# csiro-crop-informatics/biokanga

Measured on AMD Instinct MI355X. Metric: aligned reads/s (SAM-identical) on 100 bp SE vs GRCh38, 1->8 MI355X, higher is better.
Workload: dtype u8

## Files before the change

### biokanga_amd/csrc/bk_ctx_int.h

```cpp
#pragma once
#include <atomic>
#include <thread>
#include <hip/hip_runtime.h>

#include <cstdio>
#include <cstring>
#include <functional>
#include <string>
#include <utility>
#include <vector>

#include "bk_device.h"
#include "bk_devbuf.h"
#include "bk_stage.h"

#define HIP_TRY(expr)                                                                              \
    do {                                                                                           \
        hipError_t e__ = (expr);                                                                   \
        if (e__ != hipSuccess) {                                                                   \
            fprintf(stderr, "biokanga_amd: %s failed: %s (%s:%d)\n", #expr, hipGetErrorString(e__), __FILE__, __LINE__); \
            return e__ == hipErrorOutOfMemory ? BK_ERR_MEM : BK_ERR_INTERNAL;                      \
        }                                                                                          \
    } while (0)
#define BK_TRY(expr) do { const int rc__ = (expr); if (rc__) return rc__; } while (0)
// ... 150 lines not shown
    bk_timing timing{};
    std::vector<hipEvent_t> ev_pool;
    std::vector<uint64_t> loci_offs;
    std::vector<bk_loci> loci;
    std::vector<bk_loci_trims> loci_trims;
    std::vector<bk_seg2> seg2;
};


namespace bk {
struct DevReads {
    const uint8_t *bases = nullptr;
    const uint64_t *offs = nullptr;
    const uint32_t *lens = nullptr;
    const uint32_t *words = nullptr;
    const bk_nbase *exc = nullptr;
    uint64_t n_exc = 0;
};
int engine_align_device(bk_ctx *c, const DevReads &in, uint32_t nreads, bk_hit *d_out, hipStream_t s, uint32_t maxlen_known = 0, uint32_t minlen_known = 0);
void release_swin(bk_ctx *c);
void drop_swin(bk_ctx *c);
int engine_pair_device(bk_ctx *c, const DevReads &in, uint32_t n_pairs, bk_hit *d_hits, uint32_t maxlen, const bk_pe_params *pe, hipStream_t s,
                       bk_seg2 *seg2_host = nullptr, bk_seg2 *seg2_dev = nullptr);
int engine_prepare_packed(bk_ctx *c, const uint16_t *d_lens16, uint32_t nreads, uint64_t n_words, const bk_nbase *d_exc, uint64_t n_exc,
                          uint32_t *d_lens32, uint64_t *d_offs, uint32_t *maxlen, uint32_t *minlen, hipStream_t s);
}

namespace bk {
hipError_t dev_zero_now(void *p, size_t bytes);
int upload_host(void *d_dst, const void *h_src, size_t bytes, int device);
int upload_file(void *d_dst, int fd, uint64_t file_ofs, size_t bytes, int device);
bool host_is_pinned(const void *p);

std::vector<uint32_t> seq_len_by_id(const bk_ctx *c);
void gather_split(uint64_t total_bytes, uint32_t n, const std::function<void(uint32_t, uint32_t)> &part);
template <class SpanOf> inline void gather_reads(uint8_t *dst, const uint64_t *dst_ofs, const uint8_t *src, uint64_t total_bytes, uint32_t n, SpanOf span_of)
{
    gather_split(total_bytes, n, [&](uint32_t lo, uint32_t hi) {
        for (uint32_t t = lo; t < hi; t++) {
            if (dst_ofs[t] == ~0ULL) continue;
            const std::pair<uint64_t, uint32_t> sp = span_of(t);
            memcpy(dst + dst_ofs[t], src + sp.first, sp.second);
        }
    });
}
}
```

### biokanga_amd/csrc/bk_engine.cpp

```cpp
#include "bk_engine_int.h"
#include "bk_iv_slot.h"
#include "bk_wave_form.h"

namespace bk {
int size_heavy_scratch(bk_ctx *c)
{
    int slides = std::max(1, (c->cfg.slides_per100 * c->max_read_len + 99) / 100);
    uint64_t worst = c->cfg.max_iter ? (uint64_t)slides * (uint64_t)c->cfg.max_iter : kNodeCap;
    if (worst > kNodeCap) worst = kNodeCap;
    uint32_t ts = 1024;
    while (ts < 2 * worst) ts <<= 1;
    uint32_t slots = 4096;
    while ((uint64_t)slots * ts * 8 > (16ULL << 30) && slots > 64) slots >>= 1;
    if (c->hs.htab && c->hs.tab_size == ts && c->hs.n_slots == slots) return BK_OK;
    BatchBufs &m = c->buf;
    m.htab.reset();
    m.slot_epoch.reset();
    c->hs = HeavyScratch{};
    HIP_TRY(m.htab.ensure((size_t)slots * ts));
    HIP_TRY(m.slot_epoch.ensure(slots));
    launch_fill_u64(m.htab.get(), (uint64_t)slots * ts, 0ULL, c->stream);
    HIP_TRY(hipGetLastError());
    HIP_TRY(hipMemsetAsync(m.slot_epoch.get(), 0, (size_t)slots * 4, c->stream));
    HIP_TRY(hipStreamSynchronize(c->stream));
// ... 668 lines not shown
        case Span::Prep: c->timing.ms_prep += m; c->timing.ms_other += m; break;
        case Span::Other: c->timing.ms_other += m; break;
        }
    }
    return BK_OK;
}


}

using namespace bk;

int bk::engine_align_device(bk_ctx *c, const DevReads &in, uint32_t nreads, bk_hit *d_out, hipStream_t s, uint32_t maxlen_known, uint32_t minlen_known)
{
    return align_device(c, in, nreads, d_out, s, maxlen_known, false, minlen_known);
}

namespace {
struct CastU64 {
    __host__ __device__ unsigned long long operator()(const uint32_t &v) const { return (unsigned long long)v; }
};
}

int bk::engine_prepare_packed(bk_ctx *c, const uint16_t *d_lens16, uint32_t nreads, uint64_t n_words, const bk_nbase *d_exc, uint64_t n_exc,
                              uint32_t *d_lens32, uint64_t *d_offs, uint32_t *maxlen, uint32_t *minlen, hipStream_t s)
{
    launch_widen_lens(d_lens16, nreads, d_lens32, (unsigned long long *)d_offs, s);
    HIP_TRY(hipGetLastError());
    size_t need = 0;
    HIP_TRY(bk::prim::exclusive_sum(nullptr, need, (unsigned long long *)d_offs, (unsigned long long *)d_offs, (size_t)nreads, s));
    if (need > c->buf.scan_tmp.cap()) {
        HIP_TRY(hipStreamSynchronize(s));
        HIP_TRY(c->buf.scan_tmp.ensure(need + 256));
    }
    size_t tb = c->buf.scan_tmp.cap();
    HIP_TRY(bk::prim::exclusive_sum(c->buf.scan_tmp.get(), tb, (unsigned long long *)d_offs, (unsigned long long *)d_offs, (size_t)nreads, s));
    HIP_TRY(hipMemsetAsync(c->fixed.ctr_aux.get(), 0, 32, s));
    launch_packed_extent(d_offs, d_lens32, nreads, c->fixed.ctr_aux.get(), s);
    launch_check_exc(d_exc, n_exc, d_lens32, nreads, reinterpret_cast<uint32_t *>(c->fixed.ctr_aux.get() + 2), s);
    launch_min_len(d_lens32, nreads, reinterpret_cast<uint32_t *>(c->fixed.ctr_aux.get() + 3), s);
    HIP_TRY(hipGetLastError());
    unsigned long long h[4] = {0, 0, 0, 0};
    HIP_TRY(hipMemcpyAsync(h, c->fixed.ctr_aux.get(), 32, hipMemcpyDeviceToHost, s));
    HIP_TRY(hipStreamSynchronize(s));
    if (h[0] != n_words || h[1] > (unsigned long long)kMaxReadLenAbs || (uint32_t)h[2] != 0) return BK_ERR_PARAMS;
    *maxlen = (uint32_t)h[1];
    *minlen = min_len_of((uint32_t)h[3]);
    return BK_OK;
}

int bk::engine_pair_device(bk_ctx *c, const DevReads &in, uint32_t n_pairs, bk_hit *d_hits, uint32_t maxlen, const bk_pe_params *pe, hipStream_t s,
                           bk_seg2 *seg2_host, bk_seg2 *seg2_dev)
{
    const uint32_t nreads = 2 * n_pairs;
    const uint32_t wpr = words_per_read(maxlen);
    const uint32_t ivc = c->cap_iv_cores ? c->cap_iv_cores : iv_cores_for(c, maxlen);
    BK_TRY(batch_scratch_or_release_swin(c, nreads, wpr, 0, ivc));
    const DevBatch b = make_batch(c, in, 0, nreads, wpr, c->cap_iv_cores, d_hits);
    if (c->params.min_chimeric_len > 0 && !seg2_host && !seg2_dev) return BK_ERR_PARAMS;
    bk_seg2 *d_seg2 = seg2_dev;
    if (!d_seg2 && seg2_host) {
        BK_TRY(ensure_seg2(c, nreads));
        d_seg2 = c->buf.seg2.get();
        HIP_TRY(hipMemcpyAsync(d_seg2, seg2_host, (size_t)nreads * sizeof(bk_seg2), hipMemcpyHostToDevice, s));
    }
    HIP_TRY(hipMemsetAsync(c->fixed.small.get(), 0, kSmallWords * 4, s));
    launch_pe(c->ix, c->cfg, b, pe->pe_mode, pe->pair_min_len, pe->pair_max_len, pe->pair_strand ? 1 : 0, d_hits, n_pairs,
              c->buf.heavy.get(), c->fixed.small.get() + kSmCount, c->h_small.get() + kSmCount, d_seg2, c->params.min_chimeric_len, maxlen > 512 ? 1 : 0, c->buf.chrom_accept.get(), c->n_chrom_accept, s);
    HIP_TRY(hipGetLastError());
    if (seg2_host && !seg2_dev) HIP_TRY(hipMemcpyAsync(seg2_host, d_seg2, (size_t)nreads * sizeof(bk_seg2), hipMemcpyDeviceToHost, s));
// ... 195 lines not shown
    for (unsigned t = 0; t < nt; t++) {
        for (const bk_nbase &e : found[t]) { if (total < exc_cap) exc[total] = e; total++; }
    }
    *n_exc = total;
    return total > exc_cap ? BK_ERR_MEM : BK_OK;
}

int bk_align_batch_packed(bk_ctx *c, const uint32_t *words, uint64_t n_words, const uint16_t *lens, uint32_t nreads, const bk_nbase *exc,
                          uint64_t n_exc, bk_hit *out)
{
    if (!c || (nreads && (!lens || !out)) || (n_words && !words) || (n_exc && !exc)) return BK_ERR_PARAMS;
    if (!nreads) return BK_OK;
    HIP_TRY(hipSetDevice(c->device));
    hipStream_t s = c->stream;
    static_assert(kPackedPadWords >= kNwLongest, "packed read words must be padded by the widest register-window family");
    BatchBufs &m = c->buf;
    HIP_TRY(m.in_words.ensure(n_words + kPackedPadWords));
    HIP_TRY(m.in_exc.ensure(n_exc));
    BK_TRY(ensure_in_reads(c, nreads, true));
    if (n_words) HIP_TRY(hipMemcpyAsync(m.in_words.get(), words, n_words * 4, hipMemcpyHostToDevice, s));
    HIP_TRY(hipMemcpyAsync(m.in_lens16.get(), lens, (size_t)nreads * 2, hipMemcpyHostToDevice, s));
    if (n_exc) HIP_TRY(hipMemcpyAsync(m.in_exc.get(), exc, n_exc * sizeof(bk_nbase), hipMemcpyHostToDevice, s));
    uint32_t maxlen = 0, minlen = 0;
    BK_TRY(engine_prepare_packed(c, m.in_lens16.get(), nreads, n_words, m.in_exc.get(), n_exc, m.in_lens.get(), m.in_offs.get(), &maxlen, &minlen, s));
    DevReads in;
    in.offs = m.in_offs.get(); in.lens = m.in_lens.get(); in.words = m.in_words.get(); in.exc = m.in_exc.get(); in.n_exc = n_exc;
    BK_TRY(align_device(c, in, nreads, m.in_out.get(), s));
    HIP_TRY(hipMemcpy(out, m.in_out.get(), (size_t)nreads * sizeof(bk_hit), hipMemcpyDeviceToHost));
    return BK_OK;
}

int bk_pair_batch(bk_ctx *c, const uint8_t *bases, const uint64_t *offs, const uint32_t *lens, uint32_t n_pairs, bk_hit *hits,
                  const bk_pe_params *pe)
{
    return bk_pair_batch_seg2(c, bases, offs, lens, n_pairs, hits, nullptr, pe);
}

int bk_pair_batch_seg2(bk_ctx *c, const uint8_t *bases, const uint64_t *offs, const uint32_t *lens, uint32_t n_pairs, bk_hit *hits,
                       bk_seg2 *seg2, const bk_pe_params *pe)
{
    if (!c || !pe || (n_pairs && (!bases || !offs || !lens || !hits))) return BK_ERR_PARAMS;
    if (c->params.min_chimeric_len > 0 && n_pairs && !seg2) return BK_ERR_PARAMS;
    if (pe->pe_mode < 1 || pe->pe_mode > 4 || pe->pair_min_len < 1 || pe->pair_max_len < pe->pair_min_len) return BK_ERR_PARAMS;
    if (!n_pairs) return BK_OK;
    if (n_pairs > 0x7fffffffu) return BK_ERR_PARAMS;
    HIP_TRY(hipSetDevice(c->device));
    const uint32_t nreads = 2 * n_pairs;
// ... 118 lines not shown
```

### biokanga_amd/csrc/bk_engine_int.h

```cpp
#pragma once
#include <hip/hip_runtime.h>
#include <fcntl.h>
#include <unistd.h>
#include "bk_prim.h"

#include <algorithm>
#include <cstdio>
#include <cstdlib>
#include <ctime>
#include <cstring>
#include <map>
#include <mutex>
#include <string>
#include <atomic>
#include <thread>
#include <type_traits>
#include <vector>

#include <dlfcn.h>
#include <rccl/rccl.h>

#include "bk_ctx_int.h"
#include "bk_phase_plan.h"
#include "bk_cpus.h"
#include "bk_wait.h"
#include "bk_env.h"
#include "sfx_file.h"


namespace bk {
void launch_pack_target(const uint8_t *seq, uint64_t n, uint64_t *tgt4, uint64_t nwords, hipStream_t s);
void launch_pack_target2(const uint64_t *tgt4, uint64_t nwords4, uint64_t *tgt2, unsigned int *nflag32, int flag_shift, hipStream_t s);
void launch_split_sa5(const uint8_t *sa5, uint64_t n, uint32_t *lo, uint8_t *hi, hipStream_t s);
void launch_build_ktab(const DevIndex &ix, void *tab, int k, bool tab64, hipStream_t s, uint64_t i0 = 0, uint64_t i1 = 0, unsigned long long *starts = nullptr, bool pairs = false);
void launch_fill_ktab2_y(void *tab2, const uint32_t *k2, uint64_t n_entries, hipStream_t s, const uint32_t *sa_elem = nullptr);
void launch_max_len(const uint32_t *lens, uint32_t n, uint32_t *out, hipStream_t s);
void launch_min_len(const uint32_t *lens, uint32_t n, uint32_t *out, hipStream_t s);
void launch_widen_lens(const uint16_t *lens16, uint32_t n, uint32_t *lens32, unsigned long long *nwords, hipStream_t s);
void launch_check_exc(const bk_nbase *exc, uint64_t n_exc, const uint32_t *lens, uint32_t n_reads, uint32_t *bad, hipStream_t s);
void launch_packed_extent(const uint64_t *offs, const uint32_t *lens, uint32_t n, unsigned long long *out, hipStream_t s);
void launch_snp_pileup(const DevIndex &ix, const uint8_t *bases, const uint64_t *offs, const uint32_t *id2idx, const bk_snp_aln *alns, uint64_t n_alns,
                       uint32_t *planes, hipStream_t s);
void launch_site_octamers(const DevIndex &ix, const bk_site_req *reqs, uint64_t n, int32_t rel_ofs, bk_site_res *out, hipStream_t s);
void launch_primer_correct(const DevIndex &ix, const bk_primer_req *reqs, uint64_t n, bk_primer_res *out, hipStream_t s);
void launch_snp_gather(const DevIndex &ix, const uint32_t *planes, uint64_t g0, uint32_t n, uint32_t *out, hipStream_t s);
void launch_snp_centroids(const DevIndex &ix, const uint32_t *planes, uint64_t g0, uint32_t chrom_len, uint32_t min_reads, uint32_t *hist, hipStream_t s);
void launch_snp_sites(const DevIndex &ix, const uint32_t *planes, uint64_t g0, uint32_t chrom_len, uint32_t min_reads, double min_prop,
                      bk_snp_site *sites, uint32_t cap, uint32_t *n_sites, unsigned long long *totals, hipStream_t s);
void launch_count_seqs(const bk_hit *out, uint32_t n, const uint32_t *id2idx, uint32_t n_ent, unsigned long long *counts, hipStream_t s);
void launch_fill_u64(unsigned long long *p, uint64_t n, unsigned long long v, hipStream_t s);
void launch_prep(const DevAlignCfg &cfg, const DevBatch &b, uint32_t *act, uint32_t *act_cnt, uint32_t *cmax, uint32_t *stage,
                 uint32_t *stripe_cnt, hipStream_t s, const PrepSearch0 *s0 = nullptr);
void launch_search(const DevIndex &ix, const DevAlignCfg &cfg, const DevBatch &b, const uint32_t *act, uint32_t n_act,
                   int phase, int cmax, int nstr, int lazy, hipStream_t s);
void launch_build_isa(const uint32_t *sa, uint64_t n, uint32_t *isa, hipStream_t s, uint64_t i0 = 0, uint64_t i1 = 0);
void launch_build_swin(const DevIndex &ix, void *swin, int words, hipStream_t s);
void launch_swin_breaks(const DevIndex &ix, const int *w, int n_levels, unsigned long long *const *brk, uint64_t a, uint64_t e, uint64_t n_words,
                        const unsigned long long *starts, hipStream_t s);
void launch_swin_cover(const unsigned long long *brk, uint64_t n, uint32_t max_run, uint32_t min_run, uint32_t *flags, uint64_t n_blocks, int first_level, hipStream_t s);
void launch_pack_ktab64(const uint64_t *tab, uint64_t n_entries, uint32_t *off, uint64_t *hi, uint32_t *overflow, hipStream_t s);
void launch_count_nonzero(const uint32_t *flags, uint64_t n, unsigned long long *count, hipStream_t s);
// ... 114 lines not shown
```

### biokanga_amd/csrc/bk_prep.hip

```cpp
#include "bk_dev_search_a.h"
#include "bk_plan_table.h"

namespace bk {


__global__ void __launch_bounds__(256) k_compact_lists(CompactJobs J)
{
    const int li = blockIdx.y;
    __shared__ uint32_t s_pre[kListStripes + 1];
    if (threadIdx.x < 64) {
        uint32_t run = 0;
        for (int s0 = 0; s0 < kListStripes; s0 += 64) {
            uint32_t v = J.set.cnt[(s0 + threadIdx.x) * 16 + li];
            for (int off = 1; off < 64; off <<= 1) { uint32_t u = __shfl_up(v, off); if ((int)threadIdx.x >= off) v += u; }
            s_pre[s0 + threadIdx.x + 1] = run + v;
            run += __shfl(v, 63);
        }
        if (threadIdx.x == 0) s_pre[0] = 0;
    }
    __syncthreads();
    const uint32_t tot = s_pre[kListStripes], old = *J.total[li];
    const uint32_t *__restrict__ stage = J.set.stage[li];
    uint32_t *__restrict__ dense = J.dense[li];
    for (uint32_t i = blockIdx.x * 256 + threadIdx.x; i < tot; i += gridDim.x * 256) {
// ... 146 lines not shown
            unsigned long long *p = reinterpret_cast<unsigned long long *>(b.rd4 + ((uint64_t)rr * 2 + st) * b.wpr + w);
            atomicAnd(p, ~m);
            atomicOr(p, code16 & m);
        }
    }
}

__global__ void __launch_bounds__(256) k_check_exc(const bk_nbase *__restrict__ exc, uint64_t n_exc, const uint32_t *__restrict__ lens, uint32_t n_reads,
                                                   uint32_t *__restrict__ bad)
{
    const uint64_t i = (uint64_t)blockIdx.x * blockDim.x + threadIdx.x;
    if (i >= n_exc) return;
    const bk_nbase e = exc[i];
    bool ok = e.read < n_reads && e.code >= 4 && e.code <= 7;
    if (ok) ok = (uint32_t)e.pos + e.run < lens[e.read];
    if (ok && i > 0) {
        const bk_nbase q = exc[i - 1];
        ok = q.read < e.read || (q.read == e.read && (uint32_t)q.pos + q.run < e.pos);
    }
    if (!ok) atomicAdd(bad, 1u);
}

__global__ void __launch_bounds__(256) k_widen_lens(const uint16_t *__restrict__ lens16, uint32_t n, uint32_t *__restrict__ lens32,
                                                    unsigned long long *__restrict__ nwords)
{
    const uint32_t i = blockIdx.x * blockDim.x + threadIdx.x;
    if (i >= n) return;
    const uint32_t l = lens16[i];
    lens32[i] = l;
    nwords[i] = (l + 15) >> 4;
}

__global__ void __launch_bounds__(256) k_packed_extent(const uint64_t *__restrict__ offs, const uint32_t *__restrict__ lens, uint32_t n,
                                                       unsigned long long *__restrict__ out)
{
    unsigned long long e = 0, l = 0;
    for (uint64_t i = (uint64_t)blockIdx.x * blockDim.x + threadIdx.x; i < n; i += (uint64_t)gridDim.x * blockDim.x) {
        const unsigned long long len = lens[i], end = offs[i] + ((len + 15) >> 4);
        e = end > e ? end : e;
        l = len > l ? len : l;
    }
    for (int off = 32; off > 0; off >>= 1) {
        const unsigned long long e2 = __shfl_down(e, off), l2 = __shfl_down(l, off);
        e = e2 > e ? e2 : e;
        l = l2 > l ? l2 : l;
    }
    if ((threadIdx.x & 63) == 0) {
        if (e) atomicMax(out + 0, e);
        if (l) atomicMax(out + 1, l);
    }
}

void launch_packed_extent(const uint64_t *offs, const uint32_t *lens, uint32_t n, unsigned long long *out, hipStream_t s)
{
    unsigned blocks = (n + 255) / 256;
    if (blocks > 2048) blocks = 2048;
    if (n) hipLaunchKernelGGL(k_packed_extent, dim3(blocks), dim3(256), 0, s, offs, lens, n, out);
}

void launch_widen_lens(const uint16_t *lens16, uint32_t n, uint32_t *lens32, unsigned long long *nwords, hipStream_t s)
{
    if (n) hipLaunchKernelGGL(k_widen_lens, dim3((n + 255) / 256), dim3(256), 0, s, lens16, n, lens32, nwords);
}

void launch_check_exc(const bk_nbase *exc, uint64_t n_exc, const uint32_t *lens, uint32_t n_reads, uint32_t *bad, hipStream_t s)
{
    if (n_exc) hipLaunchKernelGGL(k_check_exc, dim3((unsigned)((n_exc + 255) / 256)), dim3(256), 0, s, exc, n_exc, lens, n_reads, bad);
}

__global__ void __launch_bounds__(256) k_pack_reads(DevBatch b, const uint32_t *__restrict__ pairs, uint32_t n_pairs)
{
    const uint32_t wpr = b.wpr;
    const uint32_t per_read = 2 * wpr;
    const uint32_t rpb = 256 / per_read;
    const uint32_t lr = threadIdx.x / per_read;
    if (lr >= rpb) return;
    uint64_t r = (uint64_t)blockIdx.x * rpb + lr;
    if (pairs != nullptr) {
        if (r >= 2ULL * n_pairs) return;
        r = 2ULL * pairs[r >> 1] + (r & 1);
    }
    if (r >= b.n_reads) return;
    const uint32_t rem = threadIdx.x - lr * per_read;
    const uint32_t st = rem >= wpr ? 1 : 0, w = rem - st * wpr;
    int len = (int)b.lens[r];
// ... 505 lines not shown
```

### biokanga_amd/csrc/bk_stream.cpp

```cpp
#include <hip/hip_runtime.h>
#include "bk_prim.h"

#include <algorithm>
#include <cstdlib>
#include <condition_variable>
#include <deque>
#include <map>
#include <mutex>
#include <thread>

#include "bk_ctx_int.h"
#include "bk_wave_form.h"
#include "bk_wait.h"
#include "bk_env.h"

namespace {

struct CastU64 {
    __host__ __device__ unsigned long long operator()(const uint32_t &v) const { return (unsigned long long)v; }
};

__global__ void __launch_bounds__(256) k_extent(const uint64_t *__restrict__ offs, const uint32_t *__restrict__ lens, uint32_t n,
                                                unsigned long long nbases, unsigned long long *__restrict__ out)
{
// ... 25 lines not shown
    uint64_t ticket = 0;
    const uint8_t *bases = nullptr;
    uint64_t nbases = 0;
    const uint64_t *offs = nullptr;
    const uint32_t *lens = nullptr;
    const uint32_t *words = nullptr;
    uint64_t n_words = 0;
    const uint16_t *lens16 = nullptr;
    const bk_nbase *exc = nullptr;
    uint64_t n_exc = 0;
    uint32_t n = 0;
    bk_hit *out = nullptr;
    bool dev = false;
    const uint8_t *d_bases = nullptr;
    const uint64_t *d_offs = nullptr;
    const uint32_t *d_lens = nullptr;
    bk_hit *d_out = nullptr;
    hipEvent_t ev_in = nullptr;
    ~Job() { if (ev_in) (void)hipEventDestroy(ev_in); }
    int slot = 0;
    int rc = BK_OK;
    bool done = false;
    double t_submit = 0, t_done = 0;
    std::vector<uint64_t> loci_offs;
    std::vector<bk_loci> loci;
    std::vector<bk_loci_trims> loci_trims;
    std::vector<bk_seg2> seg2;
};

struct Slot {
    bk::DevBuf<uint8_t> d_bases;
    bk::DevBuf<uint16_t> d_lens16;
    bk::DevBuf<bk_nbase> d_exc;
    bk::DevBuf<uint64_t> d_offs;
    bk::DevBuf<uint32_t> d_lens;
    bk::DevBuf<bk_hit> d_out;
    hipEvent_t ev_up = nullptr, ev_al = nullptr;
};

using bk::now_s;

}

struct bk_stream {
    bk_ctx *ctx = nullptr;
    int depth = 0;
    uint32_t max_reads = 0;
    uint64_t max_bases = 0;
    uint64_t max_words = 0;
    std::vector<Slot> slots;
    hipStream_t s_up = nullptr, s_al = nullptr, s_dn = nullptr;
    bk::DevBuf<uint8_t> d_scan_tmp;
    size_t scan_tmp_bytes = 0;
    bk::DevBuf<unsigned long long> d_ext;
    bk::PinBuf<unsigned long long> h_ext;
    std::thread t_up, t_al, t_dn;
    hipEvent_t ev_w_al = nullptr, ev_w_dn = nullptr;
    std::mutex mu;
    std::condition_variable cv;
    std::deque<Job *> q_up, q_al, q_dn;
    std::map<uint64_t, Job *> jobs;
    uint64_t next_ticket = 1, n_done = 0;
    bool stop = false, list_modes = false, has_pe = false, span_open = false;
    bk_pe_params pe{};
    bk_stream_stats stats{};
    double t_first_submit = 0, t_last_done = 0;

    void fail(Job *j, int rc) { if (j->rc == BK_OK) j->rc = rc; }
    static int rc_of(hipError_t e) { return e == hipSuccess ? BK_OK : (e == hipErrorOutOfMemory ? BK_ERR_MEM : BK_ERR_INTERNAL); }

    Job *pop(std::deque<Job *> &q)
    {
        std::unique_lock<std::mutex> lk(mu);
        cv.wait(lk, [&] { return stop || !q.empty(); });
        if (q.empty()) return nullptr;
        Job *j = q.front();
        q.pop_front();
        return j;
    }
    void push(std::deque<Job *> &q, Job *j)
    {
        { std::lock_guard<std::mutex> lk(mu); q.push_back(j); }
        cv.notify_all();
    }

    void run_upload()
    {
        (void)hipSetDevice(ctx->device);
        while (Job *j = pop(q_up)) {
            Slot &sl = slots[j->slot];
            hipError_t e = hipSuccess;
            if (j->dev) { push(q_al, j); continue; }
            if (j->n && j->lens16) {
                const size_t wb = (size_t)j->n_words * 4;
                if (wb) {
                    if (bk::host_is_pinned(j->words)) e = hipMemcpyAsync(sl.d_bases.get(), j->words, wb, hipMemcpyHostToDevice, s_up);
                    else if (bk::upload_host(sl.d_bases.get(), j->words, wb, ctx->device) != BK_OK) e = hipErrorUnknown;
                }
                if (e == hipSuccess) e = hipMemcpyAsync(sl.d_lens16.get(), j->lens16, (size_t)j->n * 2, hipMemcpyHostToDevice, s_up);
                if (e == hipSuccess && j->n_exc > sl.d_exc.cap()) e = sl.d_exc.ensure(j->n_exc + j->n_exc / 4 + 1024);
                if (e == hipSuccess && j->n_exc) e = hipMemcpyAsync(sl.d_exc.get(), j->exc, (size_t)j->n_exc * sizeof(bk_nbase), hipMemcpyHostToDevice, s_up);
            } else if (j->n) {
                if (bk::host_is_pinned(j->bases)) e = hipMemcpyAsync(sl.d_bases.get(), j->bases, j->nbases, hipMemcpyHostToDevice, s_up);
                else if (bk::upload_host(sl.d_bases.get(), j->bases, j->nbases, ctx->device) != BK_OK) e = hipErrorUnknown;
                if (e == hipSuccess && j->offs) e = hipMemcpyAsync(sl.d_offs.get(), j->offs, (size_t)j->n * 8, hipMemcpyHostToDevice, s_up);
                if (e == hipSuccess) e = hipMemcpyAsync(sl.d_lens.get(), j->lens, (size_t)j->n * 4, hipMemcpyHostToDevice, s_up);
            }
            if (e == hipSuccess) e = hipEventRecord(sl.ev_up, s_up);
            if (e != hipSuccess) fail(j, rc_of(e));
            push(q_al, j);
        }
    }

    void run_align()
    {
        (void)hipSetDevice(ctx->device);
        const bool timing = bk::env::timing();
        double t_free = now_s();
        for (;;) {
            Job *j = pop(q_al);
            if (!j) break;
            const double t_got = now_s();
            double t_prep = t_got;
            Slot &sl = slots[j->slot];
            if (j->dev) {
                if (j->rc == BK_OK && j->n) {
                    hipError_t e = hipStreamWaitEvent(s_al, j->ev_in, 0);
                    bk::DevReads in;
                    in.bases = j->d_bases; in.offs = j->d_offs; in.lens = j->d_lens;
                    int rc = e == hipSuccess ? bk::engine_align_device(ctx, in, j->n, j->d_out, s_al, 0) : rc_of(e);
                    if (rc == BK_OK && has_pe) {
                        rc = bk::engine_pair_device(ctx, in, j->n / 2, j->d_out, (uint32_t)ctx->last_maxlen, &pe, s_al, ctx->seg2.empty() ? nullptr : ctx->seg2.data());
                    }
                    if (rc) fail(j, rc);
                    else if (list_modes) {
                        j->loci_offs.swap(ctx->loci_offs);
                        j->loci.swap(ctx->loci);
                        j->loci_trims.swap(ctx->loci_trims);
                        j->seg2.swap(ctx->seg2);
                    }
                }
                push(q_dn, j);
                t_free = now_s();
                continue;
            }
            if (j->rc == BK_OK && j->n && j->lens16) {
                hipError_t e = hipStreamWaitEvent(s_al, sl.ev_up, 0);
                uint32_t maxlen = 0, minlen = 0;
                int rc = e == hipSuccess ? bk::engine_prepare_packed(ctx, sl.d_lens16.get(), j->n, j->n_words, sl.d_exc.get(), j->n_exc, sl.d_lens.get(), sl.d_offs.get(), &maxlen, &minlen, s_al)
                                         : rc_of(e);
                t_prep = now_s();
                bk::DevReads in;
                in.offs = sl.d_offs.get(); in.lens = sl.d_lens.get(); in.words = reinterpret_cast<const uint32_t *>(sl.d_bases.get()); in.exc = sl.d_exc.get(); in.n_exc = j->n_exc;
                if (rc == BK_OK) rc = bk::engine_align_device(ctx, in, j->n, sl.d_out.get(), s_al, maxlen, minlen);
                if (rc == BK_OK && has_pe) rc = bk::engine_pair_device(ctx, in, j->n / 2, sl.d_out.get(), maxlen, &pe, s_al, ctx->seg2.empty() ? nullptr : ctx->seg2.data());
                if (rc) fail(j, rc);
                else if (list_modes) {
                    j->loci_offs.swap(ctx->loci_offs);
                    j->loci.swap(ctx->loci);
                    j->loci_trims.swap(ctx->loci_trims);
                    j->seg2.swap(ctx->seg2);
                }
                if (j->rc == BK_OK) {
                    e = hipEventRecord(sl.ev_al, s_al);
                    if (e != hipSuccess) fail(j, rc_of(e));
                }
            } else if (j->rc == BK_OK && j->n) {
                hipError_t e = hipStreamWaitEvent(s_al, sl.ev_up, 0);
                if (e == hipSuccess && !j->offs) {
                    size_t tb = scan_tmp_bytes;
                    rocprim::transform_iterator<const uint32_t *, CastU64, unsigned long long> in(sl.d_lens.get(), CastU64());
                    e = bk::prim::exclusive_sum(d_scan_tmp.get(), tb, in, (unsigned long long *)sl.d_offs.get(), (size_t)j->n, s_al);
                }
                if (e == hipSuccess) e = hipMemsetAsync(d_ext.get(), 0, 24, s_al);
                if (e == hipSuccess) {
                    unsigned blocks = (j->n + 255) / 256;
                    if (blocks > 2048) blocks = 2048;
                    hipLaunchKernelGGL(k_extent, dim3(blocks), dim3(256), 0, s_al, sl.d_offs.get(), sl.d_lens.get(), j->n, (unsigned long long)j->nbases, d_ext.get());
                    e = hipGetLastError();
                }
                if (e == hipSuccess) e = hipMemcpyAsync(h_ext.get(), d_ext.get(), 24, hipMemcpyDeviceToHost, s_al);
                if (e == hipSuccess) e = bk::wait_stream(s_al, ev_w_al);
                if (e != hipSuccess) fail(j, rc_of(e));
                else if (h_ext.get()[0] > j->nbases || h_ext.get()[1] > (unsigned long long)bk::kMaxReadLenAbs) fail(j, BK_ERR_PARAMS);
                const uint32_t maxlen = (uint32_t)h_ext.get()[1], minlen = bk::min_len_of((uint32_t)h_ext.get()[2]);
                if (j->rc == BK_OK) {
                    bk::DevReads in;
                    in.bases = sl.d_bases.get(); in.offs = sl.d_offs.get(); in.lens = sl.d_lens.get();
                    int rc = bk::engine_align_device(ctx, in, j->n, sl.d_out.get(), s_al, maxlen, minlen);
                    if (rc == BK_OK && has_pe) rc = bk::engine_pair_device(ctx, in, j->n / 2, sl.d_out.get(), maxlen, &pe, s_al, ctx->seg2.empty() ? nullptr : ctx->seg2.data());
                    if (rc) fail(j, rc);
                    else if (list_modes) {
                        j->loci_offs.swap(ctx->loci_offs);
                        j->loci.swap(ctx->loci);
                    j->loci_trims.swap(ctx->loci_trims);
                        j->seg2.swap(ctx->seg2);
                    }
                }
                if (j->rc == BK_OK) {
                    e = hipEventRecord(sl.ev_al, s_al);
                    if (e != hipSuccess) fail(j, rc_of(e));
                }
            }
            if (ctx->debug || timing)
                fprintf(stderr, "bk: stream batch of %u reads: waited %.2f ms for it, prepared in %.2f ms, aligned in %.2f ms\n", j->n, 1e3 * (t_got - t_free),
                        1e3 * (t_prep - t_got), 1e3 * (now_s() - t_prep));
            push(q_dn, j);
            t_free = now_s();
        }
    }

    void run_download()
    {
        (void)hipSetDevice(ctx->device);
        while (Job *j = pop(q_dn)) {
            Slot &sl = slots[j->slot];
            if (j->rc != BK_OK) {
                (void)hipStreamSynchronize(s_up);
                (void)hipStreamSynchronize(s_al);
                (void)hipStreamSynchronize(s_dn);
            } else if (j->dev) {
            } else if (j->n) {
                hipError_t e = hipStreamWaitEvent(s_dn, sl.ev_al, 0);
                if (e == hipSuccess) e = hipMemcpyAsync(j->out, sl.d_out.get(), (size_t)j->n * sizeof(bk_hit), hipMemcpyDeviceToHost, s_dn);
                if (e == hipSuccess) e = bk::wait_stream(s_dn, ev_w_dn);
                if (e != hipSuccess) fail(j, rc_of(e));
            }
            {
                std::lock_guard<std::mutex> lk(mu);
// ... 38 lines not shown
    if (p && hipHostUnregister(p) != hipSuccess) (void)hipGetLastError();
}

void bk_stream_destroy(bk_stream *s)
{
    if (!s) return;
    {
        std::unique_lock<std::mutex> lk(s->mu);
        s->cv.wait(lk, [&] { return s->n_done + 1 == s->next_ticket; });
        s->stop = true;
    }
    s->cv.notify_all();
    if (s->t_up.joinable()) s->t_up.join();
    if (s->t_al.joinable()) s->t_al.join();
    if (s->t_dn.joinable()) s->t_dn.join();
    (void)hipSetDevice(s->ctx->device);
    for (Slot &sl : s->slots) {
        if (sl.ev_up) (void)hipEventDestroy(sl.ev_up);
        if (sl.ev_al) (void)hipEventDestroy(sl.ev_al);
    }
    if (s->s_up) (void)hipStreamDestroy(s->s_up);
    if (s->s_al) (void)hipStreamDestroy(s->s_al);
    if (s->s_dn) (void)hipStreamDestroy(s->s_dn);
    if (s->ev_w_al) (void)hipEventDestroy(s->ev_w_al);
    if (s->ev_w_dn) (void)hipEventDestroy(s->ev_w_dn);
    for (auto &kv : s->jobs) delete kv.second;
    delete s;
}

static int stream_create(bk_stream **out, bk_ctx *ctx, uint32_t max_batch_reads, uint64_t max_batch_bases, uint64_t max_batch_words, int depth, const bk_pe_params *pe);

int bk_stream_create(bk_stream **out, bk_ctx *ctx, uint32_t max_batch_reads, uint64_t max_batch_bases, int depth, const bk_pe_params *pe)
{
    return stream_create(out, ctx, max_batch_reads, max_batch_bases, 0, depth, pe);
}

int bk_stream_create_packed(bk_stream **out, bk_ctx *ctx, uint32_t max_batch_reads, uint64_t max_batch_words, int depth, const bk_pe_params *pe)
{
    if (!max_batch_words) return BK_ERR_PARAMS;
    return stream_create(out, ctx, max_batch_reads, 0, max_batch_words, depth, pe);
}

static int stream_create(bk_stream **out, bk_ctx *ctx, uint32_t max_batch_reads, uint64_t max_batch_bases, uint64_t max_batch_words, int depth, const bk_pe_params *pe)
{
    const bool packed_only = max_batch_words != 0;
    if (packed_only) max_batch_bases = 16 * max_batch_words;
    if (!out || !ctx || !max_batch_reads || !max_batch_bases || depth < 1 || depth > 8) return BK_ERR_PARAMS;
    if (pe && (pe->pe_mode < 1 || pe->pe_mode > 4 || pe->pair_min_len < 1 || pe->pair_max_len < pe->pair_min_len)) return BK_ERR_PARAMS;
    *out = nullptr;
    HIP_TRY(hipSetDevice(ctx->device));
    bk_stream *s = new bk_stream();
    s->ctx = ctx;
    s->depth = depth;
    s->max_reads = max_batch_reads;
    s->max_bases = max_batch_bases;
    s->max_words = max_batch_words;
    s->list_modes = ctx->params.max_ml > 1 || ctx->params.micro_indel_len > 0 || ctx->params.splice_junct_len > 0 || ctx->params.min_chimeric_len > 0;
    if (pe) { s->has_pe = true; s->pe = *pe; }
    s->slots.resize((size_t)depth);
    hipError_t e = hipStreamCreateWithFlags(&s->s_up, hipStreamNonBlocking);
    if (e == hipSuccess) e = hipStreamCreateWithFlags(&s->s_al, hipStreamNonBlocking);
    if (e == hipSuccess) e = hipStreamCreateWithFlags(&s->s_dn, hipStreamNonBlocking);
    if (e == hipSuccess) e = bk::make_wait_event(&s->ev_w_al);
    if (e == hipSuccess) e = bk::make_wait_event(&s->ev_w_dn);
    auto alloc_slots = [&]() {
        hipError_t e2 = hipSuccess;
        for (Slot &sl : s->slots) {
            const uint64_t bytes = packed_only ? 4ULL * max_batch_words : std::max<uint64_t>(max_batch_bases, max_batch_bases / 4 + 4ULL * max_batch_reads);
            if (e2 == hipSuccess) e2 = sl.d_bases.ensure(bytes + 64 + 4ULL * bk::kPackedPadWords);
            if (e2 == hipSuccess) e2 = sl.d_lens16.ensure(max_batch_reads);
            if (e2 == hipSuccess) e2 = sl.d_offs.ensure(max_batch_reads);
            if (e2 == hipSuccess) e2 = sl.d_lens.ensure(max_batch_reads);
            if (e2 == hipSuccess) e2 = sl.d_out.ensure(max_batch_reads);
        }
        return e2;
    };
    if (e == hipSuccess) {
        e = alloc_slots();
        if (e == hipErrorOutOfMemory && ctx->image.swin.get()) {
            (void)hipGetLastError();
            for (Slot &sl : s->slots) sl = Slot{};
            bk::release_swin(ctx);
            e = alloc_slots();
        }
    }
    for (Slot &sl : s->slots) {
        if (e == hipSuccess) e = hipEventCreateWithFlags(&sl.ev_up, hipEventDisableTiming);
        if (e == hipSuccess) e = hipEventCreateWithFlags(&sl.ev_al, hipEventDisableTiming);
    }
    if (e == hipSuccess) {
        rocprim::transform_iterator<const uint32_t *, CastU64, unsigned long long> in(nullptr, CastU64());
        e = bk::prim::exclusive_sum(nullptr, s->scan_tmp_bytes, in, (unsigned long long *)nullptr, (size_t)max_batch_reads, s->s_al);
    }
    if (e == hipSuccess) e = s->d_scan_tmp.ensure(s->scan_tmp_bytes ? s->scan_tmp_bytes : 16);
    if (e == hipSuccess) e = s->d_ext.ensure(3);
    if (e == hipSuccess) e = s->h_ext.ensure(3);
    if (e != hipSuccess) {
        fprintf(stderr, "biokanga_amd: bk_stream_create: %s\n", hipGetErrorString(e));
        s->next_ticket = 1;
        bk_stream_destroy(s);
        return e == hipErrorOutOfMemory ? BK_ERR_MEM : BK_ERR_INTERNAL;
    }
    s->t_up = std::thread([s] { s->run_upload(); });
    s->t_al = std::thread([s] { s->run_align(); });
    s->t_dn = std::thread([s] { s->run_download(); });
    *out = s;
    return BK_OK;
}

int bk_stream_submit(bk_stream *s, const uint8_t *bases, uint64_t nbases, const uint64_t *offs, const uint32_t *lens, uint32_t nreads,
                     bk_hit *out, uint64_t *ticket)
{
    if (!s || !ticket || (nreads && (!bases || !lens || !out))) return BK_ERR_PARAMS;
    if (nreads > s->max_reads || nbases > s->max_bases || s->max_words || (s->has_pe && (nreads & 1))) return BK_ERR_PARAMS;
    Job *j = new Job();
// ... 150 lines not shown
```

Measured before the change: 787.3 million.

## Move read-batch intake prep to upload thread and fuse length stats kernel

Moves per-batch preparation (length widening, offset scan, extent and exception checks, and the blocking host readback) from the align thread onto the upload thread and stream, so the align stream no longer stalls on a host sync before each alignment. The widen-lens kernel is made grid-stride and now also computes the max length, the min length (via inverted max) and the last word count, replacing the separate packed-extent and min-len kernels. The host reads these stats plus the final offset instead of a 32-byte counter block. This adds per-stream scratch and a wait event, and the upload thread now blocks on a device sync per batch.

```diff
diff --git a/biokanga_amd/csrc/bk_ctx_int.h b/biokanga_amd/csrc/bk_ctx_int.h
--- a/biokanga_amd/csrc/bk_ctx_int.h
+++ b/biokanga_amd/csrc/bk_ctx_int.h
@@ -196,7 +196,15 @@
 void drop_swin(bk_ctx *c);
 int engine_pair_device(bk_ctx *c, const DevReads &in, uint32_t n_pairs, bk_hit *d_hits, uint32_t maxlen, const bk_pe_params *pe, hipStream_t s,
                        bk_seg2 *seg2_host = nullptr, bk_seg2 *seg2_dev = nullptr);
-int engine_prepare_packed(bk_ctx *c, const uint16_t *d_lens16, uint32_t nreads, uint64_t n_words, const bk_nbase *d_exc, uint64_t n_exc,
+struct IntakeScratch {
+    void *scan_tmp = nullptr;
+    size_t scan_tmp_bytes = 0;
+    uint32_t *d_words = nullptr;
+    unsigned long long *h_line = nullptr;
+    hipEvent_t ev_wait = nullptr;
+};
+size_t packed_scan_bytes(uint32_t nreads, hipStream_t s);
+int engine_prepare_packed(const IntakeScratch &x,const uint16_t *d_lens16, uint32_t nreads, uint64_t n_words, const bk_nbase *d_exc, uint64_t n_exc,
                           uint32_t *d_lens32, uint64_t *d_offs, uint32_t *maxlen, uint32_t *minlen, hipStream_t s);
 }
 
diff --git a/biokanga_amd/csrc/bk_engine.cpp b/biokanga_amd/csrc/bk_engine.cpp
--- a/biokanga_amd/csrc/bk_engine.cpp
+++ b/biokanga_amd/csrc/bk_engine.cpp
@@ -714,30 +714,32 @@
 };
 }
 
-int bk::engine_prepare_packed(bk_ctx *c, const uint16_t *d_lens16, uint32_t nreads, uint64_t n_words, const bk_nbase *d_exc, uint64_t n_exc,
+size_t bk::packed_scan_bytes(uint32_t nreads, hipStream_t s)
+{
+    size_t need = 0;
+    if (bk::prim::exclusive_sum(nullptr, need, (unsigned long long *)nullptr, (unsigned long long *)nullptr, (size_t)nreads, s) != hipSuccess) { (void)hipGetLastError(); return 0; }
+    return need;
+}
+
+int bk::engine_prepare_packed(const IntakeScratch &x, const uint16_t *d_lens16, uint32_t nreads, uint64_t n_words, const bk_nbase *d_exc, uint64_t n_exc,
                               uint32_t *d_lens32, uint64_t *d_offs, uint32_t *maxlen, uint32_t *minlen, hipStream_t s)
 {
-    launch_widen_lens(d_lens16, nreads, d_lens32, (unsigned long long *)d_offs, s);
+    if (!nreads || packed_scan_bytes(nreads, s) > x.scan_tmp_bytes) return BK_ERR_INTERNAL;
+    HIP_TRY(hipMemsetAsync(x.d_words, 0, 16, s));
+    launch_widen_lens_stats(d_lens16, nreads, d_lens32, (unsigned long long *)d_offs, x.d_words, s);
     HIP_TRY(hipGetLastError());
-    size_t need = 0;
-    HIP_TRY(bk::prim::exclusive_sum(nullptr, need, (unsigned long long *)d_offs, (unsigned long long *)d_offs, (size_t)nreads, s));
-    if (need > c->buf.scan_tmp.cap()) {
-        HIP_TRY(hipStreamSynchronize(s));
-        HIP_TRY(c->buf.scan_tmp.ensure(need + 256));
-    }
-    size_t tb = c->buf.scan_tmp.cap();
-    HIP_TRY(bk::prim::exclusive_sum(c->buf.scan_tmp.get(), tb, (unsigned long long *)d_offs, (unsigned long long *)d_offs, (size_t)nreads, s));
-    HIP_TRY(hipMemsetAsync(c->fixed.ctr_aux.get(), 0, 32, s));
-    launch_packed_extent(d_offs, d_lens32, nreads, c->fixed.ctr_aux.get(), s);
-    launch_check_exc(d_exc, n_exc, d_lens32, nreads, reinterpret_cast<uint32_t *>(c->fixed.ctr_aux.get() + 2), s);
-    launch_min_len(d_lens32, nreads, reinterpret_cast<uint32_t *>(c->fixed.ctr_aux.get() + 3), s);
+    size_t tb = x.scan_tmp_bytes;
+    HIP_TRY(bk::prim::exclusive_sum(x.scan_tmp, tb, (unsigned long long *)d_offs, (unsigned long long *)d_offs, (size_t)nreads, s));
+    launch_check_exc(d_exc, n_exc, d_lens32, nreads, x.d_words + 3, s);
     HIP_TRY(hipGetLastError());
-    unsigned long long h[4] = {0, 0, 0, 0};
-    HIP_TRY(hipMemcpyAsync(h, c->fixed.ctr_aux.get(), 32, hipMemcpyDeviceToHost, s));
-    HIP_TRY(hipStreamSynchronize(s));
-    if (h[0] != n_words || h[1] > (unsigned long long)kMaxReadLenAbs || (uint32_t)h[2] != 0) return BK_ERR_PARAMS;
-    *maxlen = (uint32_t)h[1];
-    *minlen = min_len_of((uint32_t)h[3]);
+    HIP_TRY(hipMemcpyAsync(x.h_line, x.d_words, 16, hipMemcpyDeviceToHost, s));
+    HIP_TRY(hipMemcpyAsync(x.h_line + 2, d_offs + (nreads - 1), 8, hipMemcpyDeviceToHost, s));
+    HIP_TRY(x.ev_wait ? bk::wait_stream(s, x.ev_wait) : hipStreamSynchronize(s));
+    uint32_t w[4];
+    memcpy(w, x.h_line, 16);
+    if (x.h_line[2] + w[2] != n_words || w[0] > (uint32_t)kMaxReadLenAbs || w[3] != 0) return BK_ERR_PARAMS;
+    *maxlen = w[0];
+    *minlen = min_len_of(w[1]);
     return BK_OK;
 }
 
@@ -979,7 +981,15 @@
     HIP_TRY(hipMemcpyAsync(m.in_lens16.get(), lens, (size_t)nreads * 2, hipMemcpyHostToDevice, s));
     if (n_exc) HIP_TRY(hipMemcpyAsync(m.in_exc.get(), exc, n_exc * sizeof(bk_nbase), hipMemcpyHostToDevice, s));
     uint32_t maxlen = 0, minlen = 0;
-    BK_TRY(engine_prepare_packed(c, m.in_lens16.get(), nreads, n_words, m.in_exc.get(), n_exc, m.in_lens.get(), m.in_offs.get(), &maxlen, &minlen, s));
+    const size_t need = packed_scan_bytes(nreads, s);
+    if (need > m.scan_tmp.cap()) {
+        HIP_TRY(hipStreamSynchronize(s));
+        HIP_TRY(m.scan_tmp.ensure(need + 256));
+    }
+    unsigned long long h[3] = {0, 0, 0};
+    IntakeScratch x;
+    x.scan_tmp = m.scan_tmp.get(); x.scan_tmp_bytes = m.scan_tmp.cap(); x.d_words = reinterpret_cast<uint32_t *>(c->fixed.ctr_aux.get()); x.h_line = h;
+    BK_TRY(engine_prepare_packed(x, m.in_lens16.get(), nreads, n_words, m.in_exc.get(), n_exc, m.in_lens.get(), m.in_offs.get(), &maxlen, &minlen, s));
     DevReads in;
     in.offs = m.in_offs.get(); in.lens = m.in_lens.get(); in.words = m.in_words.get(); in.exc = m.in_exc.get(); in.n_exc = n_exc;
     BK_TRY(align_device(c, in, nreads, m.in_out.get(), s));
diff --git a/biokanga_amd/csrc/bk_engine_int.h b/biokanga_amd/csrc/bk_engine_int.h
--- a/biokanga_amd/csrc/bk_engine_int.h
+++ b/biokanga_amd/csrc/bk_engine_int.h
@@ -37,6 +37,7 @@
 void launch_max_len(const uint32_t *lens, uint32_t n, uint32_t *out, hipStream_t s);
 void launch_min_len(const uint32_t *lens, uint32_t n, uint32_t *out, hipStream_t s);
 void launch_widen_lens(const uint16_t *lens16, uint32_t n, uint32_t *lens32, unsigned long long *nwords, hipStream_t s);
+void launch_widen_lens_stats(const uint16_t *lens16, uint32_t n, uint32_t *lens32, unsigned long long *nwords, uint32_t *stats, hipStream_t s);
 void launch_check_exc(const bk_nbase *exc, uint64_t n_exc, const uint32_t *lens, uint32_t n_reads, uint32_t *bad, hipStream_t s);
 void launch_packed_extent(const uint64_t *offs, const uint32_t *lens, uint32_t n, unsigned long long *out, hipStream_t s);
 void launch_snp_pileup(const DevIndex &ix, const uint8_t *bases, const uint64_t *offs, const uint32_t *id2idx, const bk_snp_aln *alns, uint64_t n_alns,
diff --git a/biokanga_amd/csrc/bk_prep.hip b/biokanga_amd/csrc/bk_prep.hip
--- a/biokanga_amd/csrc/bk_prep.hip
+++ b/biokanga_amd/csrc/bk_prep.hip
@@ -192,13 +192,35 @@
 }
 
 __global__ void __launch_bounds__(256) k_widen_lens(const uint16_t *__restrict__ lens16, uint32_t n, uint32_t *__restrict__ lens32,
-                                                    unsigned long long *__restrict__ nwords)
-{
-    const uint32_t i = blockIdx.x * blockDim.x + threadIdx.x;
-    if (i >= n) return;
-    const uint32_t l = lens16[i];
-    lens32[i] = l;
-    nwords[i] = (l + 15) >> 4;
+                                                    unsigned long long *__restrict__ nwords, uint32_t *__restrict__ stats)
+{
+    __shared__ uint32_t s_max, s_inv;
+    if (threadIdx.x == 0) { s_max = 0; s_inv = 0; }
+    __syncthreads();
+    uint32_t mx = 0, inv = 0;
+    for (uint64_t i = (uint64_t)blockIdx.x * blockDim.x + threadIdx.x; i < n; i += (uint64_t)gridDim.x * blockDim.x) {
+        const uint32_t l = lens16[i];
+        lens32[i] = l;
+        nwords[i] = (l + 15) >> 4;
+        mx = l > mx ? l : mx;
+        inv = ~l > inv ? ~l : inv;
+        if (stats != nullptr && i == (uint64_t)n - 1) stats[2] = (l + 15) >> 4;
+    }
+    if (stats == nullptr) return;
+    for (int off = 32; off > 0; off >>= 1) {
+        const uint32_t m2 = __shfl_down(mx, off), i2 = __shfl_down(inv, off);
+        mx = m2 > mx ? m2 : mx;
+        inv = i2 > inv ? i2 : inv;
+    }
+    if ((threadIdx.x & 63) == 0) {
+        if (mx) atomicMax(&s_max, mx);
+        if (inv) atomicMax(&s_inv, inv);
+    }
+    __syncthreads();
+    if (threadIdx.x == 0) {
+        if (s_max) atomicMax(stats + 0, s_max);
+        if (s_inv) atomicMax(stats + 1, s_inv);
+    }
 }
 
 __global__ void __launch_bounds__(256) k_packed_extent(const uint64_t *__restrict__ offs, const uint32_t *__restrict__ lens, uint32_t n,
@@ -228,9 +250,16 @@
     if (n) hipLaunchKernelGGL(k_packed_extent, dim3(blocks), dim3(256), 0, s, offs, lens, n, out);
 }
 
+void launch_widen_lens_stats(const uint16_t *lens16, uint32_t n, uint32_t *lens32, unsigned long long *nwords, uint32_t *stats, hipStream_t s)
+{
+    uint32_t blocks = (n + 255) / 256;
+    if (blocks > 2048) blocks = 2048;
+    if (n) hipLaunchKernelGGL(k_widen_lens, dim3(blocks), dim3(256), 0, s, lens16, n, lens32, nwords, stats);
+}
+
 void launch_widen_lens(const uint16_t *lens16, uint32_t n, uint32_t *lens32, unsigned long long *nwords, hipStream_t s)
 {
-    if (n) hipLaunchKernelGGL(k_widen_lens, dim3((n + 255) / 256), dim3(256), 0, s, lens16, n, lens32, nwords);
+    launch_widen_lens_stats(lens16, n, lens32, nwords, nullptr, s);
 }
 
 void launch_check_exc(const bk_nbase *exc, uint64_t n_exc, const uint32_t *lens, uint32_t n_reads, uint32_t *bad, hipStream_t s)
diff --git a/biokanga_amd/csrc/bk_stream.cpp b/biokanga_amd/csrc/bk_stream.cpp
--- a/biokanga_amd/csrc/bk_stream.cpp
+++ b/biokanga_amd/csrc/bk_stream.cpp
@@ -71,6 +71,8 @@
     int rc = BK_OK;
     bool done = false;
     double t_submit = 0, t_done = 0;
+    uint32_t maxlen = 0, minlen = 0;
+    double t_intake = 0;
     std::vector<uint64_t> loci_offs;
     std::vector<bk_loci> loci;
     std::vector<bk_loci_trims> loci_trims;
@@ -104,7 +106,7 @@
     bk::DevBuf<unsigned long long> d_ext;
     bk::PinBuf<unsigned long long> h_ext;
     std::thread t_up, t_al, t_dn;
-    hipEvent_t ev_w_al = nullptr, ev_w_dn = nullptr;
+    hipEvent_t ev_w_up = nullptr, ev_w_al = nullptr, ev_w_dn = nullptr;
     std::mutex mu;
     std::condition_variable cv;
     std::deque<Job *> q_up, q_al, q_dn;
@@ -136,6 +138,7 @@
     void run_upload()
     {
         (void)hipSetDevice(ctx->device);
+        const bool timing = bk::env::timing() || ctx->debug;
         while (Job *j = pop(q_up)) {
             Slot &sl = slots[j->slot];
             hipError_t e = hipSuccess;
@@ -155,10 +158,46 @@
                 if (e == hipSuccess && j->offs) e = hipMemcpyAsync(sl.d_offs.get(), j->offs, (size_t)j->n * 8, hipMemcpyHostToDevice, s_up);
                 if (e == hipSuccess) e = hipMemcpyAsync(sl.d_lens.get(), j->lens, (size_t)j->n * 4, hipMemcpyHostToDevice, s_up);
             }
+            if (e == hipSuccess && j->n) {
+                if (timing) (void)bk::wait_stream(s_up, ev_w_up);
+                const double t0 = now_s();
+                const int rc = intake(j, sl);
+                j->t_intake = now_s() - t0;
+                if (rc) fail(j, rc);
+            }
             if (e == hipSuccess) e = hipEventRecord(sl.ev_up, s_up);
             if (e != hipSuccess) fail(j, rc_of(e));
             push(q_al, j);
         }
+    }
+
+    int intake(Job *j, Slot &sl)
+    {
+        if (j->lens16) {
+            bk::IntakeScratch x;
+            x.scan_tmp = d_scan_tmp.get(); x.scan_tmp_bytes = scan_tmp_bytes; x.d_words = reinterpret_cast<uint32_t *>(d_ext.get()); x.h_line = h_ext.get(); x.ev_wait = ev_w_up;
+            return bk::engine_prepare_packed(x, sl.d_lens16.get(), j->n, j->n_words, sl.d_exc.get(), j->n_exc, sl.d_lens.get(), sl.d_offs.get(), &j->maxlen, &j->minlen, s_up);
+        }
+        hipError_t e = hipSuccess;
+        if (!j->offs) {
+            size_t tb = scan_tmp_bytes;
+            rocprim::transform_iterator<const uint32_t *, CastU64, unsigned long long> in(sl.d_lens.get(), CastU64());
+            e = bk::prim::exclusive_sum(d_scan_tmp.get(), tb, in, (unsigned long long *)sl.d_offs.get(), (size_t)j->n, s_up);
+        }
+        if (e == hipSuccess) e = hipMemsetAsync(d_ext.get(), 0, 24, s_up);
+        if (e == hipSuccess) {
+            unsigned blocks = (j->n + 255) / 256;
+            if (blocks > 2048) blocks = 2048;
+            hipLaunchKernelGGL(k_extent, dim3(blocks), dim3(256), 0, s_up, sl.d_offs.get(), sl.d_lens.get(), j->n, (unsigned long long)j->nbases, d_ext.get());
+            e = hipGetLastError();
+        }
+        if (e == hipSuccess) e = hipMemcpyAsync(h_ext.get(), d_ext.get(), 24, hipMemcpyDeviceToHost, s_up);
+        if (e == hipSuccess) e = bk::wait_stream(s_up, ev_w_up);
+        if (e != hipSuccess) return rc_of(e);
+        if (h_ext.get()[0] > j->nbases || h_ext.get()[1] > (unsigned long long)bk::kMaxReadLenAbs) return BK_ERR_PARAMS;
+        j->maxlen = (uint32_t)h_ext.get()[1];
+        j->minlen = bk::min_len_of((uint32_t)h_ext.get()[2]);
+        return BK_OK;
     }
 
     void run_align()
@@ -193,16 +232,15 @@
                 t_free = now_s();
                 continue;
             }
-            if (j->rc == BK_OK && j->n && j->lens16) {
+            if (j->rc == BK_OK && j->n) {
                 hipError_t e = hipStreamWaitEvent(s_al, sl.ev_up, 0);
-                uint32_t maxlen = 0, minlen = 0;
-                int rc = e == hipSuccess ? bk::engine_prepare_packed(ctx, sl.d_lens16.get(), j->n, j->n_words, sl.d_exc.get(), j->n_exc, sl.d_lens.get(), sl.d_offs.get(), &maxlen, &minlen, s_al)
-                                         : rc_of(e);
                 t_prep = now_s();
                 bk::DevReads in;
-                in.offs = sl.d_offs.get(); in.lens = sl.d_lens.get(); in.words = reinterpret_cast<const uint32_t *>(sl.d_bases.get()); in.exc = sl.d_exc.get(); in.n_exc = j->n_exc;
-                if (rc == BK_OK) rc = bk::engine_align_device(ctx, in, j->n, sl.d_out.get(), s_al, maxlen, minlen);
-                if (rc == BK_OK && has_pe) rc = bk::engine_pair_device(ctx, in, j->n / 2, sl.d_out.get(), maxlen, &pe, s_al, ctx->seg2.empty() ? nullptr : ctx->seg2.data());
+                in.offs = sl.d_offs.get(); in.lens = sl.d_lens.get();
+                if (j->lens16) { in.words = reinterpret_cast<const uint32_t *>(sl.d_bases.get()); in.exc = sl.d_exc.get(); in.n_exc = j->n_exc; }
+                else in.bases = sl.d_bases.get();
+                int rc = e == hipSuccess ? bk::engine_align_device(ctx, in, j->n, sl.d_out.get(), s_al, j->maxlen, j->minlen) : rc_of(e);
+                if (rc == BK_OK && has_pe) rc = bk::engine_pair_device(ctx, in, j->n / 2, sl.d_out.get(), j->maxlen, &pe, s_al, ctx->seg2.empty() ? nullptr : ctx->seg2.data());
                 if (rc) fail(j, rc);
                 else if (list_modes) {
                     j->loci_offs.swap(ctx->loci_offs);
@@ -214,46 +252,10 @@
                     e = hipEventRecord(sl.ev_al, s_al);
                     if (e != hipSuccess) fail(j, rc_of(e));
                 }
-            } else if (j->rc == BK_OK && j->n) {
-                hipError_t e = hipStreamWaitEvent(s_al, sl.ev_up, 0);
-                if (e == hipSuccess && !j->offs) {
-                    size_t tb = scan_tmp_bytes;
-                    rocprim::transform_iterator<const uint32_t *, CastU64, unsigned long long> in(sl.d_lens.get(), CastU64());
-                    e = bk::prim::exclusive_sum(d_scan_tmp.get(), tb, in, (unsigned long long *)sl.d_offs.get(), (size_t)j->n, s_al);
-                }
-                if (e == hipSuccess) e = hipMemsetAsync(d_ext.get(), 0, 24, s_al);
-                if (e == hipSuccess) {
-                    unsigned blocks = (j->n + 255) / 256;
-                    if (blocks > 2048) blocks = 2048;
-                    hipLaunchKernelGGL(k_extent, dim3(blocks), dim3(256), 0, s_al, sl.d_offs.get(), sl.d_lens.get(), j->n, (unsigned long long)j->nbases, d_ext.get());
-                    e = hipGetLastError();
-                }
-                if (e == hipSuccess) e = hipMemcpyAsync(h_ext.get(), d_ext.get(), 24, hipMemcpyDeviceToHost, s_al);
-                if (e == hipSuccess) e = bk::wait_stream(s_al, ev_w_al);
-                if (e != hipSuccess) fail(j, rc_of(e));
-                else if (h_ext.get()[0] > j->nbases || h_ext.get()[1] > (unsigned long long)bk::kMaxReadLenAbs) fail(j, BK_ERR_PARAMS);
-                const uint32_t maxlen = (uint32_t)h_ext.get()[1], minlen = bk::min_len_of((uint32_t)h_ext.get()[2]);
-                if (j->rc == BK_OK) {
-                    bk::DevReads in;
-                    in.bases = sl.d_bases.get(); in.offs = sl.d_offs.get(); in.lens = sl.d_lens.get();
-                    int rc = bk::engine_align_device(ctx, in, j->n, sl.d_out.get(), s_al, maxlen, minlen);
-                    if (rc == BK_OK && has_pe) rc = bk::engine_pair_device(ctx, in, j->n / 2, sl.d_out.get(), maxlen, &pe, s_al, ctx->seg2.empty() ? nullptr : ctx->seg2.data());
-                    if (rc) fail(j, rc);
-                    else if (list_modes) {
-                        j->loci_offs.swap(ctx->loci_offs);
-                        j->loci.swap(ctx->loci);
-                    j->loci_trims.swap(ctx->loci_trims);
-                        j->seg2.swap(ctx->seg2);
-                    }
-                }
-                if (j->rc == BK_OK) {
-                    e = hipEventRecord(sl.ev_al, s_al);
-                    if (e != hipSuccess) fail(j, rc_of(e));
-                }
             }
             if (ctx->debug || timing)
-                fprintf(stderr, "bk: stream batch of %u reads: waited %.2f ms for it, prepared in %.2f ms, aligned in %.2f ms\n", j->n, 1e3 * (t_got - t_free),
-                        1e3 * (t_prep - t_got), 1e3 * (now_s() - t_prep));
+                fprintf(stderr, "bk: stream batch of %u reads: waited %.2f ms for it, prepared in %.2f ms, aligned in %.2f ms; intake on the upload thread %.2f ms\n", j->n,
+                        1e3 * (t_got - t_free), 1e3 * (t_prep - t_got), 1e3 * (now_s() - t_prep), 1e3 * j->t_intake);
             push(q_dn, j);
             t_free = now_s();
         }
@@ -338,6 +340,7 @@
     if (s->s_up) (void)hipStreamDestroy(s->s_up);
     if (s->s_al) (void)hipStreamDestroy(s->s_al);
     if (s->s_dn) (void)hipStreamDestroy(s->s_dn);
+    if (s->ev_w_up) (void)hipEventDestroy(s->ev_w_up);
     if (s->ev_w_al) (void)hipEventDestroy(s->ev_w_al);
     if (s->ev_w_dn) (void)hipEventDestroy(s->ev_w_dn);
     for (auto &kv : s->jobs) delete kv.second;
@@ -377,6 +380,7 @@
     hipError_t e = hipStreamCreateWithFlags(&s->s_up, hipStreamNonBlocking);
     if (e == hipSuccess) e = hipStreamCreateWithFlags(&s->s_al, hipStreamNonBlocking);
     if (e == hipSuccess) e = hipStreamCreateWithFlags(&s->s_dn, hipStreamNonBlocking);
+    if (e == hipSuccess) e = bk::make_wait_event(&s->ev_w_up);
     if (e == hipSuccess) e = bk::make_wait_event(&s->ev_w_al);
     if (e == hipSuccess) e = bk::make_wait_event(&s->ev_w_dn);
     auto alloc_slots = [&]() {
@@ -406,7 +410,8 @@
     }
     if (e == hipSuccess) {
         rocprim::transform_iterator<const uint32_t *, CastU64, unsigned long long> in(nullptr, CastU64());
-        e = bk::prim::exclusive_sum(nullptr, s->scan_tmp_bytes, in, (unsigned long long *)nullptr, (size_t)max_batch_reads, s->s_al);
+        e = bk::prim::exclusive_sum(nullptr, s->scan_tmp_bytes, in, (unsigned long long *)nullptr, (size_t)max_batch_reads, s->s_up);
+        s->scan_tmp_bytes = std::max(s->scan_tmp_bytes, bk::packed_scan_bytes(max_batch_reads, s->s_up));
     }
     if (e == hipSuccess) e = s->d_scan_tmp.ensure(s->scan_tmp_bytes ? s->scan_tmp_bytes : 16);
     if (e == hipSuccess) e = s->d_ext.ensure(3);
```

Result: no change. 794.4 million (median of 6 runs) (+0.9%).
